# FlyCole/Dream2Real

Hardware: AMD Instinct MI355X
Metric: candidate renders scored/sec (640x360) (higher is better)
Workload: dtype bf16 + fp16 NeRF MLP operands (fp32 accumulate; the library's default: the reference's tiny-cuda-nn operand type, same MFMA rate; --opt mlp_f16=0 = bf16 operands)

## Files before the change

dream2real_amd/csrc/api.hip:

```cpp
#include <math.h>
#include <string.h>

#include <algorithm>
#include <chrono>

#include "d2r_internal.h"
#include "pngio.h"

struct d2r_clip;
int d2r_launch_preprocess(d2r_ctx *, d2r_clip *, const uint8_t *frames_dev, uint32_t n, uint32_t w, uint32_t h,
                          int rot90, uint16_t *patches_dev, float *pixel_values_dev, const void *rects_dev = nullptr,
                          const uint16_t *bg_patches_dev = nullptr, bool touched_only = false);
bool d2r_clip_l0_supported(const d2r_ctx *, const d2r_clip *);
int d2r_clip_forward(d2r_ctx *, const d2r_clip *, const uint16_t *patches_dev, uint32_t n, const float *text_dev,
                     uint32_t C, float logit_scale, float *logits_dev, float *embeds_dev, const ClipL0Reuse *reuse = nullptr);
int d2r_clip_layer0_background(d2r_ctx *, const d2r_clip *, const uint16_t *bg_patches_dev, ClipL0Reuse *out);
int d2r_launch_patchify(d2r_ctx *, const d2r_clip *, const float *pv_dev, uint32_t n, uint16_t *patches_dev);
size_t d2r_clip_patch_bytes(const d2r_clip *, uint32_t n);
int d2r_launch_eval_points(d2r_ctx *, const d2r_nerf *, const float *xyz, const float *dirs, uint32_t n, float *out);
uint32_t d2r_clip_image_size(const d2r_clip *);
uint32_t d2r_clip_proj_dim(const d2r_clip *);
uint32_t d2r_clip_max_images(const d2r_clip *);
uint32_t d2r_clip_tokens(const d2r_clip *);

// ... 104 lines not shown
    unsigned flags;
    int (*hook)(d2r_ctx *, int64_t value);
};
enum { OPT_DEV = 1,
       OPT_READ_ONLY = 2 };
#ifdef D2R_DEV
static const bool kDevBuild = true;
#else
static const bool kDevBuild = false;
#endif

static int opt_march_threads(d2r_ctx *ctx, int64_t value)
{
    if (value % 64)
        return d2r_fail(ctx, D2R_ERR_INVALID, "march_threads must be 0 (auto) or a multiple of 64 up to " + std::to_string(D2R_MARCH_THREADS) + " (the size the marcher was compiled for)");
    return D2R_OK;
}

static int opt_timing(d2r_ctx *ctx, int64_t)
{
    ctx->ev_used = 0;
    ctx->ev_pairs.clear();
    return D2R_OK;
}

static const Option g_options[] = {
    {"chunk", &d2r_ctx::chunk, Option::RANGE, 1, 16384},
    {"march_compact", &d2r_ctx::march_compact, Option::RANGE, 0, 1},
    {"refill_min", &d2r_ctx::refill_min, Option::RANGE, 1, 64},
    {"ln_fold", &d2r_ctx::ln_fold, Option::RANGE, 0, 4},
    {"gemm_nsplit", &d2r_ctx::gemm_nsplit, Option::FREE},
    {"prep_reuse", &d2r_ctx::prep_reuse, Option::FLAG},
    {"cls_last", &d2r_ctx::cls_last, Option::FLAG},
    {"vit_fp8", &d2r_ctx::vit_fp8, Option::FLAG},
    {"l0_reuse", &d2r_ctx::l0_reuse, Option::FLAG},
    {"attn_rem", &d2r_ctx::attn_rem, Option::RANGE, 0, 4},
    {"overlap", &d2r_ctx::overlap, Option::FLAG},
    {"debug_fail_chunk", &d2r_ctx::debug_fail_chunk, Option::FREE},
    {"ray_sort", &d2r_ctx::ray_sort, Option::RANGE, 0, 1},
    {"ray_sort_log2", &d2r_ctx::ray_sort_log2, Option::RANGE, 1, 4},
    {"march_threads", &d2r_ctx::march_threads, Option::RANGE, 0, D2R_MARCH_THREADS, 0, opt_march_threads},
    {"march_threads_auto_mib", &d2r_ctx::march_threads_auto_mib, Option::RANGE, 0, 1 << 20},
    {"march_blocks", &d2r_ctx::march_blocks, Option::RANGE, 0, 65535},
    {"gemm_cfg", &d2r_ctx::gemm_cfg, Option::FREE, 0, 0, OPT_DEV},
    {"gemm_group", &d2r_ctx::gemm_group, Option::RANGE, 0, 65535, OPT_DEV},
    {"gemm_stagger", &d2r_ctx::gemm_stagger, Option::FLAG, 0, 0, OPT_DEV},
    {"gbrick_slots", &d2r_ctx::gbrick_slots, Option::RANGE, 0, 8},
    {"brick_slots_total", &d2r_ctx::brick_slots_total, Option::RANGE, 0, 8},
    {"lds_slots_max", &d2r_ctx::lds_slots_max, Option::RANGE, 0, 5},
    {"gbrick_max_mib", &d2r_ctx::gbrick_max_mib, Option::RANGE, 0, 512},
    {"mlp_f16", &d2r_ctx::mlp_f16, Option::FLAG},
    {"render_arith", &d2r_ctx::render_arith, Option::RANGE, 0, 2},
    {"bricks", &d2r_ctx::use_bricks, Option::FLAG},
    {"raygen_rect", &d2r_ctx::raygen_rect, Option::FLAG},
    {"timing", &d2r_ctx::timing, Option::RANGE, 0, 2, 0, opt_timing},
    {"march_lds_slots", &d2r_ctx::last_march_nb, Option::FREE, 0, 0, OPT_READ_ONLY},
    {"march_hbm_brick_slots", &d2r_ctx::last_march_ngb, Option::FREE, 0, 0, OPT_READ_ONLY},
    {"march_hbm_brick_bytes", &d2r_ctx::last_march_gbrick_bytes, Option::FREE, 0, 0, OPT_READ_ONLY},
    {"march_threads_used", &d2r_ctx::last_march_threads, Option::FREE, 0, 0, OPT_READ_ONLY},
};

static const Option *find_option(const char *key)
{
    for (const Option &o : g_options)
        if (!strcmp(key, o.key)) return (o.flags & OPT_DEV) && !kDevBuild ? nullptr : &o;
    return nullptr;
// ... 948 lines not shown
```

dream2real_amd/csrc/clip.hip:

```cpp
#include "d2r_internal.h"

#include <type_traits>

#include <math.h>
#include <stdio.h>
#include <stdlib.h>

#include <algorithm>
#include <deque>
#include <mutex>

typedef __bf16 bf16x8 __attribute__((ext_vector_type(8)));
typedef float f32x16 __attribute__((ext_vector_type(16)));
typedef float f32x4 __attribute__((ext_vector_type(4)));

struct ClipWeights {
    const uint16_t *w_patch;
    const float *cls, *pos;
    const float *pre_w, *pre_b;
    struct Layer {
        const float *ln1_w, *ln1_b, *ln2_w, *ln2_b;
        const uint16_t *w_qkv, *w_o, *w_fc1, *w_fc2;
        const float *b_qkv, *b_o, *b_fc1, *b_fc2;
        const uint16_t *wf_qkv = nullptr, *wf_fc1 = nullptr;
// ... 2246 lines not shown
}

__global__ void k_gather_cls(const float *__restrict__ X, const uint16_t *__restrict__ Xhi, const uint16_t *__restrict__ Xlo,
                             uint32_t M_pad, uint32_t T, uint32_t d, uint32_t n, float *__restrict__ X_cls, int lo8 = 0)
{
    const uint32_t i = blockIdx.x * blockDim.x + threadIdx.x;
    if (i >= n * d) return;
    const uint32_t img = i / d, c = i - img * d;
    const size_t row = (size_t)img * T;
    float v;
    if (Xhi) {
        const size_t xo = ((size_t)(c >> 6) * M_pad + row) * 64 + (c & 63);
        v = __uint_as_float((uint32_t)Xhi[xo] << 16);
        if (Xlo && lo8) v = split8_value(Xhi[xo], ((const int8_t *)Xlo)[lo8_off(M_pad, row, c)]);
        else if (Xlo) v += __uint_as_float((uint32_t)Xlo[xo] << 16);
    } else {
        v = X[row * d + c];
    }
    X_cls[i] = v;
}

__global__ void k_gather_cls_operand(const uint16_t *__restrict__ Xhi, const float2 *__restrict__ AB, uint32_t M_pad, uint32_t T,
                                     uint32_t d, uint32_t n, uint16_t *__restrict__ Xq, float2 *__restrict__ ABq)
{
    const uint32_t i = blockIdx.x * blockDim.x + threadIdx.x, per = d / 8;
    if (i >= n * per) return;
    const uint32_t img = i / per, c = (i - img * per) * 8;
    const size_t row = (size_t)img * T;
    *(uint4 *)(Xq + (size_t)img * d + c) = *(const uint4 *)(Xhi + ((size_t)(c >> 6) * M_pad + row) * 64 + (c & 63));
    if (c == 0) ABq[img] = AB[row];
}


#define HEAD_THREADS 1024
#define HEAD_NI 4
__global__ __launch_bounds__(HEAD_THREADS) void k_head(const float *__restrict__ X, const uint16_t *__restrict__ Xb,
                                                       const uint16_t *__restrict__ Xlo, uint32_t M_pad,
                                                       const uint32_t *__restrict__ pool_row, uint32_t T, uint32_t d,
                                                       const float *__restrict__ lw, const float *__restrict__ lb,
                                                       const float *__restrict__ proj, uint32_t D,
                                                       const float *__restrict__ text, uint32_t C, float logit_scale,
                                                       float *__restrict__ logits, float *__restrict__ embeds, uint32_t n_items, int lo8 = 0)
{
    __shared__ float xs[HEAD_NI][1024];
    __shared__ float es[HEAD_NI][1024];
    __shared__ float red[HEAD_NI][16];
    constexpr uint32_t NW = HEAD_THREADS / 64;
    const uint32_t tid = threadIdx.x, lane = tid & 63, wave = tid >> 6;
    const uint32_t item0 = blockIdx.x * HEAD_NI;
    const uint32_t ni = min((uint32_t)HEAD_NI, n_items - item0);
    float xv[HEAD_NI];
#pragma unroll
    for (uint32_t m = 0; m < HEAD_NI; m++) {
        xv[m] = 0.f;
        if (m < ni && tid < d) {
            const size_t xrow = (size_t)(item0 + m) * T + (pool_row ? pool_row[item0 + m] : 0u);
            const size_t xo = ((size_t)(tid >> 6) * M_pad + xrow) * 64 + (tid & 63);
            xv[m] = Xb ? __uint_as_float((uint32_t)Xb[xo] << 16) : X[xrow * d + tid];
            if (Xb && Xlo && lo8) xv[m] = split8_value(Xb[xo], ((const int8_t *)Xlo)[lo8_off(M_pad, xrow, tid)]);
            else if (Xb && Xlo) xv[m] += __uint_as_float((uint32_t)Xlo[xo] << 16);
        }
        const float s = wave_sum(xv[m]);
        if (lane == 0) red[m][wave] = s;
    }
    __syncthreads();
    float mu[HEAD_NI], dv[HEAD_NI];
// ... 340 lines not shown
        if (g * 8 < n_qt) {
            if (r == 1) hipLaunchKernelGGL((k_attention_s<1, true>), dim3(n_heads, n, 1), dim3(64), lds, ctx->stream, QKV, AO, T, d, M_pad, g * 8, q8_scales);
            else if (r == 2) hipLaunchKernelGGL((k_attention_s<2, true>), dim3(n_heads, n, 1), dim3(128), lds, ctx->stream, QKV, AO, T, d, M_pad, g * 8, q8_scales);
            else hipLaunchKernelGGL((k_attention_s<4, true>), dim3(n_heads, n, 1), dim3(256), lds, ctx->stream, QKV, AO, T, d, M_pad, g * 8, q8_scales);
        }
        return;
    }
    if (g) hipLaunchKernelGGL((k_attention_s<8>), dim3(n_heads, n, g), dim3(512), lds, ctx->stream, QKV, AO, T, d, M_pad, 0u, no_scales);
    if (g * 8 < n_qt) {
        if (r == 1) hipLaunchKernelGGL((k_attention_s<1>), dim3(n_heads, n, 1), dim3(64), lds, ctx->stream, QKV, AO, T, d, M_pad, g * 8, no_scales);
        else if (r == 2) hipLaunchKernelGGL((k_attention_s<2>), dim3(n_heads, n, 1), dim3(128), lds, ctx->stream, QKV, AO, T, d, M_pad, g * 8, no_scales);
        else hipLaunchKernelGGL((k_attention_s<4>), dim3(n_heads, n, 1), dim3(256), lds, ctx->stream, QKV, AO, T, d, M_pad, g * 8, no_scales);
    }
}

static int attention_setup(d2r_ctx *ctx, uint32_t T_pad, size_t *lds_out)
{
    const size_t attn_lds = (size_t)T_pad * 128 + (size_t)64 * (T_pad + 4) * 2;
    if (attn_lds > 160 * 1024) return d2r_fail(ctx, D2R_ERR_UNSUPPORTED, "sequence too long for the resident attention LDS layout");
    static PerDeviceOnce attn_attr;
    attn_attr.run(ctx->device, [] {
        (void)hipFuncSetAttribute((const void *)k_attention<true>, hipFuncAttributeMaxDynamicSharedMemorySize, 160 * 1024);
    });
    *lds_out = attn_lds;
    return D2R_OK;
}

static int last_block_cls(d2r_ctx *ctx, const d2r_clip_desc &D, const ClipWeights::Layer &L, uint32_t n, uint32_t T, uint32_t rows_pad,
                          const uint16_t *QKV, const uint16_t *Qc, const float *X, const uint16_t *Xhi, const uint16_t *Xlo, float *Xc,
                          uint16_t *AOc, uint16_t *Xnc, uint16_t *Hc, int lo8 = 0)
{
    const uint32_t d = D.hidden_size, mlp = D.mlp_size, items = n * D.num_heads;
    int rc;
    hipLaunchKernelGGL(k_attention_cls, dim3((items + 3) / 4), dim3(256), 0, ctx->stream, QKV, Qc, AOc, T, d, rows_pad, D.num_heads, items);
    hipLaunchKernelGGL(k_gather_cls, dim3((n * d + 255) / 256), dim3(256), 0, ctx->stream, X, Xhi, Xlo, rows_pad, T, d, n, Xc, lo8);
    if ((rc = launch_gemm<EPI_BIAS_RESID_F32>(ctx, AOc, L.w_o, L.b_o, Xc, n, d, d))) return rc;
    hipLaunchKernelGGL(k_layernorm, dim3((n + 3) / 4), dim3(256), 0, ctx->stream, Xc, L.ln2_w, L.ln2_b, Xnc, n, d);
    if ((rc = launch_gemm<EPI_BIAS_GELU_BF16>(ctx, Xnc, L.w_fc1, L.b_fc1, Hc, n, mlp, d))) return rc;
    if ((rc = launch_gemm<EPI_BIAS_RESID_F32>(ctx, Hc, L.w_fc2, L.b_fc2, Xc, n, d, mlp))) return rc;
    return D2R_OK;
}

bool d2r_clip_l0_supported(const d2r_ctx *ctx, const d2r_clip *clip)
{
    const d2r_clip_desc &D = clip->desc;
    const uint32_t g = D.image_size / D.patch_size;
    return ctx->ln_fold == 4 && D.num_layers >= 2 && g * g == clip->T - 1 && g * g <= 1024;
}

int d2r_clip_layer0_background(d2r_ctx *ctx, const d2r_clip *clip, const uint16_t *bg_patches_dev, ClipL0Reuse *out)
{
    const d2r_clip_desc &D = clip->desc;
    const uint32_t d = D.hidden_size, T = clip->T, R = round_up(T, BM);
    if (T > 1025 || D.num_layers < 1) return d2r_fail(ctx, D2R_ERR_UNSUPPORTED, "layer-0 reuse needs at most 1024 patches per image");
    const size_t b_hi = (size_t)R * d * 2, b_lo = (size_t)R * d, b_ab = (size_t)R * 8, b_qkv = (size_t)R * 3 * d * 2, b_po = (size_t)R * d * 4;
    int rc;
    if ((rc = d2r_reserve(ctx, ctx->bg_l0, b_hi + b_lo + b_ab + b_qkv + b_po + 1024))) return rc;
    uint8_t *base = (uint8_t *)ctx->bg_l0.p;
    uint16_t *hi = (uint16_t *)base;
    uint8_t *lo = base + b_hi;
    float2 *ab = (float2 *)(lo + b_lo);
    uint16_t *qkv = (uint16_t *)((uint8_t *)ab + b_ab);
    float *po = (float *)((uint8_t *)qkv + b_qkv);
    if ((rc = launch_gemm<EPI_F32>(ctx, bg_patches_dev, clip->w.w_patch, nullptr, po, T - 1, d, clip->Kp_pad))) return rc;
    hipLaunchKernelGGL(k_embed_ln, dim3((T + 3) / 4), dim3(256), 0, ctx->stream, po, clip->w.cls, clip->w.pos, clip->w.pre_w, clip->w.pre_b,
                       (float *)nullptr, T, T, d, hi, ab, (uint16_t *)lo, R, 1);
    const ClipWeights::Layer &L = clip->layers[0];
// ... 44 lines not shown
        }
        f8[l].w_qkv = out[0]; f8[l].w_o = out[1]; f8[l].w_fc1 = out[2]; f8[l].w_fc2 = out[3];
    }
    std::vector<uint32_t> bits(nl * 4);
    D2R_HIP(ctx, hipMemcpyAsync(bits.data(), amax, nl * 16, hipMemcpyDeviceToHost, ctx->stream));
    D2R_HIP(ctx, hipStreamSynchronize(ctx->stream));
    auto scale_of = [](uint32_t b) {
        const int e = (int)((b + 0x200000u) >> 23);
        const int byte = std::min(std::max(e - 8, 1), 253);
        return std::ldexp(1.0f, byte - 127);
    };
    for (size_t l = 0; l < nl; l++) {
        f8[l].s_qkv = scale_of(bits[l * 4 + 0]); f8[l].s_o = scale_of(bits[l * 4 + 1]);
        f8[l].s_fc1 = scale_of(bits[l * 4 + 2]); f8[l].s_fc2 = scale_of(bits[l * 4 + 3]);
    }
    clip->f8 = std::move(f8);
    return D2R_OK;
}

int d2r_clip_forward(d2r_ctx *ctx, const d2r_clip *clip, const uint16_t *patches_dev, uint32_t n,
                     const float *text_dev, uint32_t C, float logit_scale, float *logits_dev, float *embeds_dev,
                     const ClipL0Reuse *reuse)
{
    const d2r_clip_desc &D = clip->desc;
    const uint32_t d = D.hidden_size, T = clip->T, mlp = D.mlp_size;
    const uint32_t rows = n * T, rows_pad = round_up(rows, BM);
    const uint32_t prow = n * (T - 1);
    int rc;
    if ((rc = d2r_reserve(ctx, ctx->clipws[0], (size_t)round_up(prow, BM) * d * 4))) return rc;
    if ((rc = d2r_reserve(ctx, ctx->clipws[1], (size_t)rows_pad * d * 4))) return rc;
    if ((rc = d2r_reserve(ctx, ctx->clipws[2], (size_t)rows_pad * d * 2))) return rc;
    if ((rc = d2r_reserve(ctx, ctx->clipws[3], (size_t)rows_pad * 3 * d * 2))) return rc;
    if ((rc = d2r_reserve(ctx, ctx->clipws[4], (size_t)rows_pad * d * 2))) return rc;
    if ((rc = d2r_reserve(ctx, ctx->clipws[5], (size_t)rows_pad * mlp * 2))) return rc;
    float *patch_out = (float *)ctx->clipws[0].p, *X = (float *)ctx->clipws[1].p;
    uint16_t *Xn = (uint16_t *)ctx->clipws[2].p, *QKV = (uint16_t *)ctx->clipws[3].p;
    uint16_t *AO = (uint16_t *)ctx->clipws[4].p, *H = (uint16_t *)ctx->clipws[5].p;

    const int fold = (int)ctx->ln_fold;
    const bool l0 = reuse && reuse->rects;
    if (l0 && (!d2r_clip_l0_supported(ctx, clip) || T > reuse->bg_rows))
        return d2r_fail(ctx, D2R_ERR_INVALID, "d2r_clip_forward: layer-0 reuse requested for a model / option set that does not support it");
    uint32_t *l0_cnt = nullptr, *l0_list = nullptr;
    const uint32_t cap_pad = round_up(prow, BM);
    if (l0) {
        const PrepCache *pc = nullptr;
        if ((rc = prep_tables(ctx, (d2r_clip *)clip, reuse->w, reuse->h, 1, &pc))) return rc;
        if ((rc = d2r_reserve(ctx, ctx->l0_misc, 256 + (size_t)prow * 4 + (size_t)cap_pad * 8))) return rc;
        if ((rc = d2r_reserve(ctx, ctx->l0_a1, (size_t)cap_pad * clip->Kp_pad * 2))) return rc;
        if ((rc = d2r_reserve(ctx, ctx->l0_q2, (size_t)cap_pad * 3 * d * 2))) return rc;
        l0_cnt = (uint32_t *)ctx->l0_misc.p;
        l0_list = l0_cnt + 64;
        D2R_HIP(ctx, hipMemsetAsync(l0_cnt, 0, 4, ctx->stream));
        hipLaunchKernelGGL(k_touch_list, dim3(n), dim3(256), 0, ctx->stream, (const int4 *)reuse->rects, reuse->w, pc->R, D.image_size, D.patch_size, l0_cnt, l0_list);
        hipLaunchKernelGGL(k_gather_rows, dim3(2048), dim3(256), 0, ctx->stream, patches_dev, clip->Kp_pad, l0_list, l0_cnt, (uint16_t *)ctx->l0_a1.p);
        if (reuse->touched_out) D2R_HIP(ctx, hipMemcpyAsync(reuse->touched_out, l0_cnt, 4, hipMemcpyDeviceToDevice, ctx->stream));
        if (getenv("D2R_L0_DEBUG")) {
            uint32_t c = 0;
            (void)hipMemcpyAsync(&c, l0_cnt, 4, hipMemcpyDeviceToHost, ctx->stream);
            (void)hipStreamSynchronize(ctx->stream);
            fprintf(stderr, "[d2r l0_reuse] %u of %u patch tokens touched (%.1f %%)\n", c, prow, 100.0 * c / prow);
        }
        EpiAux a1{};
        a1.m_dev = l0_cnt;
        if ((rc = launch_gemm_cfg<EPI_F32, 4, 2, 2, 3>(ctx, (const uint16_t *)ctx->l0_a1.p, clip->w.w_patch, nullptr, patch_out, prow, d, clip->Kp_pad, a1))) return rc;
    } else if ((rc = launch_gemm<EPI_F32>(ctx, patches_dev, clip->w.w_patch, nullptr, patch_out, prow, d, clip->Kp_pad)))
        return rc;
// ... 3 lines not shown
    a_tm.a_rs = 64;
    a_tm.a_ks = (uint32_t)64 * rows_pad;
    if ((uint64_t)64 * rows_pad >= (1ull << 32)) return d2r_fail(ctx, D2R_ERR_UNSUPPORTED, "activation plane too large for 32-bit indexing");
    if (fold == 0) {
        hipLaunchKernelGGL(k_embed_ln, dim3((rows + 3) / 4), dim3(256), 0, ctx->stream, patch_out, clip->w.cls,
                           clip->w.pos, clip->w.pre_w, clip->w.pre_b, X, rows, T, d, (uint16_t *)nullptr, (float2 *)nullptr, (uint16_t *)nullptr, rows_pad);
        for (uint32_t l = 0; l < D.num_layers; l++) {
            const ClipWeights::Layer &L = clip->layers[l];
            hipLaunchKernelGGL(k_layernorm, dim3((rows + 3) / 4), dim3(256), 0, ctx->stream, X, L.ln1_w, L.ln1_b, Xn,
                               rows, d);
            if ((rc = launch_gemm<EPI_BIAS_BF16>(ctx, Xn, L.w_qkv, L.b_qkv, QKV, rows, 3 * d, d, out_tm))) return rc;
            if (cls_last && l + 1 == D.num_layers) {
                if ((rc = last_block_cls(ctx, D, L, n, T, rows_pad, QKV, nullptr, X, nullptr, nullptr, patch_out, AO, Xn, H))) return rc;
                break;
            }
            launch_attention_vision(ctx, QKV, AO, T, d, rows_pad, D.num_heads, n);
            if ((rc = launch_gemm<EPI_BIAS_RESID_F32>(ctx, AO, L.w_o, L.b_o, X, rows, d, d, a_tm))) return rc;
            hipLaunchKernelGGL(k_layernorm, dim3((rows + 3) / 4), dim3(256), 0, ctx->stream, X, L.ln2_w, L.ln2_b, Xn,
                               rows, d);
            if ((rc = launch_gemm<EPI_BIAS_GELU_BF16>(ctx, Xn, L.w_fc1, L.b_fc1, H, rows, mlp, d, out_tm))) return rc;
            if ((rc = launch_gemm<EPI_BIAS_RESID_F32>(ctx, H, L.w_fc2, L.b_fc2, X, rows, d, mlp, a_tm))) return rc;
        }
        hipLaunchKernelGGL(k_head, dim3((n + HEAD_NI - 1) / HEAD_NI), dim3(HEAD_THREADS), 0, ctx->stream, cls_last ? patch_out : X, (const uint16_t *)nullptr, (const uint16_t *)nullptr, rows_pad,
                           (const uint32_t *)nullptr, cls_last ? 1u : T, d,
                           clip->w.post_w, clip->w.post_b, clip->w.proj, D.proj_dim, text_dev, C, logit_scale, logits_dev, embeds_dev, n);
        D2R_HIP(ctx, hipGetLastError());
        return D2R_OK;
    }
    const uint32_t np = d / 64;
    if ((rc = d2r_reserve(ctx, ctx->clipws[7], (size_t)rows_pad * np * 8 + (size_t)rows_pad * 8))) return rc;
    float2 *part = (float2 *)ctx->clipws[7].p, *AB = part + (size_t)rows_pad * np;
    const bool xf32 = fold == 3, split8 = fold == 4, split = fold == 1 || split8;
    const int lo8 = split8 ? 1 : 0;
    uint16_t *Xlo = split ? (uint16_t *)X : (uint16_t *)nullptr;
    if (l0) {
        hipLaunchKernelGGL(k_bcast_x0, dim3((rows + 3) / 4), dim3(256), 0, ctx->stream, reuse->bg_hi, reuse->bg_lo, reuse->bg_ab, reuse->bg_rows, Xn,
                           (uint8_t *)Xlo, AB, rows, rows_pad, T, d);
        hipLaunchKernelGGL(k_embed_ln, dim3(std::min<uint32_t>((prow + 3) / 4, 4096u)), dim3(256), 0, ctx->stream, patch_out, clip->w.cls, clip->w.pos, clip->w.pre_w,
                           clip->w.pre_b, (float *)nullptr, rows, T, d, Xn, AB, Xlo, rows_pad, lo8, (const uint32_t *)l0_list, (const uint32_t *)l0_cnt);
    } else
    hipLaunchKernelGGL(k_embed_ln, dim3((rows + 3) / 4), dim3(256), 0, ctx->stream, patch_out, clip->w.cls, clip->w.pos,
                       clip->w.pre_w, clip->w.pre_b, xf32 ? X : (float *)nullptr, rows, T, d, Xn, AB, Xlo, rows_pad, lo8);
    EpiAux ln = out_tm, st = a_tm;
    ln.a_rs = a_tm.a_rs;
    ln.a_ks = a_tm.a_ks;
    ln.ab = AB;
    st.hm_rows = rows_pad;
    st.xb = Xn;
    st.part = part;
    st.xlo = Xlo;
    const float inv_d = 1.0f / (float)d;
    uint32_t f8_first = D.num_layers, f8_end = D.num_layers;
    uint8_t *A8 = nullptr, *SA8 = nullptr, *AOS8 = nullptr, *H8 = nullptr, *SH8 = nullptr;
    uint32_t q8_grid = 0;
    if (ctx->vit_fp8 && split8 && d % 256 == 0 && mlp % 256 == 0 && mlp >= 2 * d) {
        f8_first = l0 ? 1u : 0u;
        f8_end = cls_last ? D.num_layers - 1 : D.num_layers;
        if (f8_first < f8_end) {
            if ((rc = ensure_f8_weights(ctx, (d2r_clip *)clip))) return rc;
            const size_t rp = rows_pad;
            AOS8 = (uint8_t *)AO + rp * d;
            H8 = (uint8_t *)H;
            SH8 = H8 + rp * mlp;
            A8 = SH8 + rp * (mlp / 64);
            SA8 = A8 + rp * d;
            q8_grid = (uint32_t)ctx->n_cu * 8u;
        }
    }
    for (uint32_t l = 0; l < D.num_layers; l++) {
        const ClipWeights::Layer &L = clip->layers[l];
        ln.cs = L.cs_qkv;
        if (cls_last && l + 1 == D.num_layers) {
            EpiAux kv = ln;
            kv.cs = L.cs_qkv + d;
            if ((rc = launch_gemm<EPI_LN_BIAS_BF16>(ctx, Xn, L.wf_qkv + (size_t)d * d, L.bf_qkv + d, QKV + (size_t)d * rows_pad, rows, 2 * d, d, kv)))
                return rc;
            const uint32_t n_pad = round_up(n, BM);
            uint16_t *Xq = H, *Qc = H + (size_t)n_pad * d;
            float2 *ABq = part;
            hipLaunchKernelGGL(k_gather_cls_operand, dim3((n * (d / 8) + 255) / 256), dim3(256), 0, ctx->stream, Xn, AB, rows_pad, T, d, n, Xq, ABq);
            EpiAux lq{};
            lq.cs = L.cs_qkv;
            lq.ab = ABq;
            if ((rc = launch_gemm<EPI_LN_BIAS_BF16>(ctx, Xq, L.wf_qkv, L.bf_qkv, Qc, n, d, d, lq))) return rc;
            if ((rc = last_block_cls(ctx, D, L, n, T, rows_pad, QKV, Qc, X, xf32 ? nullptr : Xn, Xlo, patch_out, AO, Xn, H, lo8))) return rc;
            break;
        }
        if (f8_first <= l && l < f8_end) {
            const d2r_clip::F8Layer &F = clip->f8[l];
            hipLaunchKernelGGL(k_ln_q8, dim3(q8_grid), dim3(256), 0, ctx->stream, Xn, AB, L.ln1_w, L.ln1_b, rows_pad, d, A8, SA8);
            if ((rc = launch_gemm_f8<EPI_F8_BIAS_BF16>(ctx, A8, SA8, F.w_qkv, F.s_qkv, L.b_qkv, QKV, rows, 3 * d, d, out_tm))) return rc;
            launch_attention_vision(ctx, QKV, AO, T, d, rows_pad, D.num_heads, n, AOS8);
            if ((rc = launch_gemm_f8<EPI_F8_RESID_STATS_SPLIT8>(ctx, (const uint8_t *)AO, AOS8, F.w_o, F.s_o, L.b_o, Xn, rows, d, d, st))) return rc;
            hipLaunchKernelGGL(k_rowstats, dim3((rows_pad + 255) / 256), dim3(256), 0, ctx->stream, part, np, rows_pad, inv_d, AB);
            hipLaunchKernelGGL(k_ln_q8, dim3(q8_grid), dim3(256), 0, ctx->stream, Xn, AB, L.ln2_w, L.ln2_b, rows_pad, d, A8, SA8);
            EpiAux hq = out_tm;
            hq.q8 = H8;
            hq.q8_scale = SH8;
            if ((rc = launch_gemm_f8<EPI_F8_BIAS_GELU_Q8>(ctx, A8, SA8, F.w_fc1, F.s_fc1, L.b_fc1, nullptr, rows, mlp, d, hq))) return rc;
            if ((rc = launch_gemm_f8<EPI_F8_RESID_STATS_SPLIT8>(ctx, H8, SH8, F.w_fc2, F.s_fc2, L.b_fc2, Xn, rows, d, mlp, st))) return rc;
            if (l + 1 < D.num_layers)
                hipLaunchKernelGGL(k_rowstats, dim3((rows_pad + 255) / 256), dim3(256), 0, ctx->stream, part, np, rows_pad, inv_d, AB);
            continue;
        }
        if (l0 && l == 0) {
            const uint32_t planes = 3 * d / 64;
            const size_t pieces = (size_t)planes * rows * 8;
            hipLaunchKernelGGL(k_bcast_qkv, dim3((uint32_t)((pieces + 255) / 256)), dim3(256), 0, ctx->stream, reuse->bg_qkv, reuse->bg_rows, QKV, rows, rows_pad, T, planes);
            float2 *AB2 = (float2 *)((uint8_t *)ctx->l0_misc.p + 256 + (size_t)prow * 4);
            hipLaunchKernelGGL(k_gather_operand_rows, dim3(2048), dim3(256), 0, ctx->stream, Xn, AB, rows_pad, T, (const uint32_t *)l0_list, (const uint32_t *)l0_cnt,
                               AO, AB2, cap_pad, d);
            EpiAux l2 = ln;
            l2.a_ks = 64 * cap_pad;
            l2.hm_rows = cap_pad;
            l2.ab = AB2;
            l2.m_dev = l0_cnt;
            if ((rc = launch_gemm_cfg<EPI_LN_BIAS_BF16, 4, 2, 2, 3>(ctx, AO, L.wf_qkv, L.bf_qkv, ctx->l0_q2.p, prow, 3 * d, d, l2))) return rc;
            hipLaunchKernelGGL(k_scatter_qkv, dim3(8192), dim3(256), 0, ctx->stream, (const uint16_t *)ctx->l0_q2.p, cap_pad, (const uint32_t *)l0_list,
// ... 407 lines not shown
```

dream2real_amd/csrc/d2r_internal.h:

```cpp
#pragma once
#include <hip/hip_runtime.h>
#include <stdint.h>

#include <functional>
#include <memory>
#include <mutex>
#include <string>
#include <utility>
#include <vector>

#include "../../include/d2r.h"
#include "d2r_shared.h"

class D2rJobPool;
struct D2rPngBase;

#define D2R_MAX_LEVELS 16
#define D2R_MAX_DEVICES 64
#define D2R_GRID 128
#define D2R_DT 0.0016914558f
#define D2R_INV_DT (1.0f / D2R_DT)
#define D2R_CONE 0.00390625f
#define D2R_T_LINEAR (D2R_DT * 256.0f)
#define D2R_N_WFRAG 24
// ... 102 lines not shown
    uint32_t bg_w = 0, bg_h = 0;
    d2r_render_stats stats{};
    int n_cu = 256, n_xcd = 8;
    void *comm = nullptr;
    int comm_rank = 0, comm_world = 1;
    hipStream_t render_stream = nullptr, copy_stream = nullptr;
    hipEvent_t ev_fork = nullptr, ev_prep[2] = {nullptr, nullptr}, ev_clip[2] = {nullptr, nullptr},
               ev_march[2] = {nullptr, nullptr}, ev_copy[2] = {nullptr, nullptr};
    Buf patches2, frames2;
    void *frame_host[2] = {nullptr, nullptr};
    size_t frame_host_cap[2] = {0, 0};
    D2rJobPool *pool = nullptr;
    std::shared_ptr<const D2rPngBase> png_base;
    int64_t overlap = 0;
    int64_t debug_fail_chunk = -1;
    uint32_t last_chunks = 0;
    int64_t chunk = 4096;
    uint32_t last_pass = 0;
    int64_t march_blocks = 0;
    int64_t ray_sort = 1;
    int64_t ray_sort_log2 = 4;
    int64_t march_threads = 0;
    int64_t march_threads_auto_mib = 64;
    int64_t last_march_threads = 0, last_march_gbrick_bytes = 0;
    int64_t last_march_nb = 0, last_march_ngb = 0;
    int64_t refill_min = 64;
    int64_t march_compact = 1;
    int64_t ln_fold = 4;
    int64_t gemm_stagger = 0;
    int64_t gemm_group = 65535;
    int64_t gemm_nsplit = 0;
    int64_t attn_rem = 1;
    int64_t cls_last = 1;
    int64_t gemm_cfg = 0;
    int64_t mlp_f16 = 1;
    int64_t render_arith = 0;
    int64_t use_bricks = 1;
    int64_t raygen_rect = 1;
    int64_t gbrick_slots = 8;
    int64_t brick_slots_total = 7;
    int64_t lds_slots_max = 5;
    int64_t gbrick_max_mib = 512;
    int64_t timing = 0;
    std::vector<hipEvent_t> ev_pool;
    size_t ev_used = 0;
    std::vector<std::pair<int, std::pair<size_t, size_t>>> ev_pairs;
    size_t timing_begin(int kind);
    void timing_end(size_t pair);
};
enum { D2R_T_MARCH = 0, D2R_T_RAYGEN = 1, D2R_T_CLIP = 2, D2R_T_PREP = 3, D2R_T_SORT = 4,
       D2R_T_VIT_QKV = 5, D2R_T_VIT_ATTN = 6, D2R_T_VIT_OUT = 7, D2R_T_VIT_FC1 = 8, D2R_T_VIT_FC2 = 9, D2R_T_KINDS = 10 };

struct d2r_nerf {
    d2r_ctx *ctx;
    int device = 0;
    NerfParams P{};
    D2rDev<uint32_t> d_grid, d_brick_tab, d_gbrick_tab;
    D2rDev<uint64_t> d_bricks;
    D2rDev<uint4> d_wfrag;
};

struct d2r_pcd {
    int device = 0;
    uint32_t n = 0;
    D2rDev<float4> xyz;
    D2rDev<uint32_t> rgb;
// ... 42 lines not shown
```

Measured before the change: 28870.

## Fold K/V projections into CLS-only last-layer attention to skip full KV GEMM

In the last ViT layer, when only the CLS token is needed, the full K/V projection over all tokens is skipped. The CLS query is folded through the K weights into a per-head query in hidden space. Attention scores and the probability-weighted token sum are then computed directly on the normalized hidden states, and the V projection is applied once per head afterwards. This removes a large rows×2d×d GEMM in exchange for three new kernels that carry fp32 values as hi/lo bf16 splits to preserve precision, plus a larger workspace.

```diff
diff --git a/dream2real_amd/csrc/api.hip b/dream2real_amd/csrc/api.hip
--- a/dream2real_amd/csrc/api.hip
+++ b/dream2real_amd/csrc/api.hip
@@ -160,6 +160,7 @@
     {"gemm_nsplit", &d2r_ctx::gemm_nsplit, Option::FREE},
     {"prep_reuse", &d2r_ctx::prep_reuse, Option::FLAG},
     {"cls_last", &d2r_ctx::cls_last, Option::FLAG},
+    {"cls_fold", &d2r_ctx::cls_fold, Option::FLAG},
     {"vit_fp8", &d2r_ctx::vit_fp8, Option::FLAG},
     {"l0_reuse", &d2r_ctx::l0_reuse, Option::FLAG},
     {"attn_rem", &d2r_ctx::attn_rem, Option::RANGE, 0, 4},
diff --git a/dream2real_amd/csrc/clip.hip b/dream2real_amd/csrc/clip.hip
--- a/dream2real_amd/csrc/clip.hip
+++ b/dream2real_amd/csrc/clip.hip
@@ -2302,6 +2302,312 @@
 }
 
 
+#define CLSF_NI 8
+__global__ __launch_bounds__(256) void k_cls_qfold(const uint16_t *__restrict__ Qc, const uint16_t *__restrict__ Wk, const float *__restrict__ csk,
+                                                   uint32_t n, uint32_t d, uint32_t H, float *__restrict__ Qt, float *__restrict__ Cc)
+{
+    __shared__ __attribute__((aligned(16))) float qs[64][CLSF_NI];
+    const uint32_t h = blockIdx.y, i0 = blockIdx.x * CLSF_NI, tid = threadIdx.x, lane = tid & 63, np2 = d >> 1;
+    for (uint32_t idx = tid; idx < 64 * CLSF_NI; idx += 256) {
+        const uint32_t i = idx >> 6, e = idx & 63;
+        qs[e][i] = i0 + i < n ? __uint_as_float((uint32_t)Qc[(size_t)(i0 + i) * d + h * 64 + e] << 16) : 0.f;
+    }
+    __syncthreads();
+    if (tid < 64) {
+        const float cs = csk[h * 64 + lane];
+#pragma unroll
+        for (int i = 0; i < CLSF_NI; i++) {
+            const float v = wave_sum(qs[lane][i] * cs);
+            if (lane == 0 && i0 + i < n) Cc[(size_t)(i0 + i) * H + h] = v;
+        }
+    }
+    float acc[2][CLSF_NI][2];
+#pragma unroll
+    for (int t = 0; t < 2; t++)
+#pragma unroll
+        for (int i = 0; i < CLSF_NI; i++) acc[t][i][0] = acc[t][i][1] = 0.f;
+    const uint16_t *Wh = Wk + (size_t)h * 64 * d;
+#pragma unroll 4
+    for (uint32_t e = 0; e < 64; e++) {
+        const float4 qa = *(const float4 *)&qs[e][0], qb = *(const float4 *)&qs[e][4];
+        const float q[CLSF_NI] = {qa.x, qa.y, qa.z, qa.w, qb.x, qb.y, qb.z, qb.w};
+#pragma unroll
+        for (int t = 0; t < 2; t++) {
+            const uint32_t pi = tid + 256 * t;
+            if (pi < np2) {
+                const uint32_t wv = *(const uint32_t *)(Wh + (size_t)e * d + 2 * pi);
+                const float w0 = bf_lo(wv), w1 = bf_hi(wv);
+#pragma unroll
+                for (int i = 0; i < CLSF_NI; i++) {
+                    acc[t][i][0] = fmaf(q[i], w0, acc[t][i][0]);
+                    acc[t][i][1] = fmaf(q[i], w1, acc[t][i][1]);
+                }
+            }
+        }
+    }
+#pragma unroll
+    for (int t = 0; t < 2; t++) {
+        const uint32_t pi = tid + 256 * t;
+        if (pi >= np2) continue;
+#pragma unroll
+        for (int i = 0; i < CLSF_NI; i++)
+            if (i0 + i < n) *(float2 *)(Qt + ((size_t)(i0 + i) * H + h) * d + 2 * pi) = make_float2(acc[t][i][0], acc[t][i][1]);
+    }
+}
+
+static size_t cls_fold_lds(uint32_t d, uint32_t nw) { return (size_t)32 * (d + 8) * 2 + (size_t)nw * 2 * 64 * 16 + 32 * 16 * 4 + 2 * 16 * 4 + 4 * 16 * 4 + 16 * 4; }
+
+__global__ __launch_bounds__(512) void k_attention_cls_fold(const uint16_t *__restrict__ Xn, const float2 *__restrict__ AB,
+                                                            const float *__restrict__ Qt, const float *__restrict__ Cc, uint32_t T, uint32_t d,
+                                                            uint32_t M_pad, uint32_t H, float *__restrict__ P, float *__restrict__ SB)
+{
+    extern __shared__ __attribute__((aligned(16))) uint8_t cf_lds[];
+    const uint32_t tid = threadIdx.x, lane = tid & 63, w = tid >> 6, NT = blockDim.x, NW = NT >> 6, img = blockIdx.x;
+    const uint32_t xst = d + 8;
+    uint16_t *xs = (uint16_t *)cf_lds;
+    float4 *part = (float4 *)(xs + 32 * xst);
+    float *wl = (float *)(part + NW * 128);
+    float *tmax = wl + 512;
+    float *red = tmax + 32;
+    float *scb = red + 64;
+    const uint32_t hb = 4 * (lane >> 4), tl = lane & 15, kq = 8 * (lane >> 4);
+    const uint32_t KS = d >> 5, NP = 4 * d;
+    const size_t row0 = (size_t)img * T;
+    union U8 { uint4 u; bf16x8 v; };
+    bf16x8 qhi[4], qlo[4];
+#pragma unroll
+    for (int i = 0; i < 4; i++) {
+        const uint32_t kk = 4 * w + i;
+        float4 v0 = make_float4(0.f, 0.f, 0.f, 0.f), v1 = v0;
+        if (kk < KS && tl < H) {
+            const float *qp = Qt + ((size_t)img * H + tl) * d + kk * 32 + kq;
+            v0 = *(const float4 *)qp;
+            v1 = *(const float4 *)(qp + 4);
+        }
+        const uint32_t h0 = pack2(v0.x, v0.y), h1 = pack2(v0.z, v0.w), h2 = pack2(v1.x, v1.y), h3 = pack2(v1.z, v1.w);
+        U8 th, tq;
+        th.u = make_uint4(h0, h1, h2, h3);
+        tq.u = make_uint4(pack2(v0.x - bf_lo(h0), v0.y - bf_hi(h0)), pack2(v0.z - bf_lo(h1), v0.w - bf_hi(h1)),
+                          pack2(v1.x - bf_lo(h2), v1.y - bf_hi(h2)), pack2(v1.z - bf_lo(h3), v1.w - bf_hi(h3)));
+        qhi[i] = th.v;
+        qlo[i] = tq.v;
+    }
+    float ch[4];
+#pragma unroll
+    for (int r = 0; r < 4; r++) ch[r] = hb + r < H ? Cc[(size_t)img * H + hb + r] : 0.f;
+    float acc0[16], acc1[16];
+#pragma unroll
+    for (int h = 0; h < 16; h++) { acc0[h] = 0.f; acc1[h] = 0.f; }
+    float mine[4], ls[4], lb[4];
+#pragma unroll
+    for (int r = 0; r < 4; r++) { mine[r] = -INFINITY; ls[r] = 0.f; lb[r] = 0.f; }
+    const bool colok = tid < (d >> 1);
+    typedef unsigned u32x4 __attribute__((ext_vector_type(4)));
+    u32x4 pf[8];
+    f32x2 abn[2] = {f32x2{0.f, 0.f}, f32x2{0.f, 0.f}};
+#define CLS_FOLD_ISSUE(C0)                                                                                                             \
+    {                                                                                                                                  \
+        _Pragma("unroll") for (int i = 0; i < 8; i++) {                                                                                \
+            const uint32_t idx = tid + i * NT;                                                                                         \
+            if (idx < NP)                                                                                                              \
+                pf[i] = *(const u32x4 *)(Xn +((size_t)(idx >> 8) * M_pad + row0 + min((C0) + ((idx >> 3) & 31), T - 1)) * 64 + (idx & 7) * 8); \
+        }                                                                                                                              \
+        if (w < 2) abn[0] = *(const f32x2 *)(AB + row0 + min((C0) + 16 * w + tl, T - 1));                                              \
+        if (w + NW < 2) abn[1] = *(const f32x2 *)(AB + row0 + min((C0) + 16 * (w + NW) + tl, T - 1));                                  \
+    }
+    CLS_FOLD_ISSUE(0u)
+    for (uint32_t c0 = 0; c0 < T; c0 += 32) {
+#pragma unroll
+        for (int i = 0; i < 8; i++) {
+            const uint32_t idx = tid + i * NT;
+            if (idx < NP) *(u32x4 *)(xs + ((idx >> 3) & 31) * xst + (idx >> 8) * 64 + (idx & 7) * 8) = pf[i];
+        }
+        const float2 ab[2] = {make_float2(abn[0][0], abn[0][1]), make_float2(abn[1][0], abn[1][1])};
+        __syncthreads();
+        if (c0 + 32 < T) CLS_FOLD_ISSUE(c0 + 32)
+#pragma unroll
+        for (int tile = 0; tile < 2; tile++) {
+            f32x4 sh = {0.f, 0.f, 0.f, 0.f}, sl = sh;
+            if (c0 + 16 * tile < T) {
+                const uint16_t *bp = xs + (16 * tile + tl) * xst + kq;
+#pragma unroll
+                for (int i = 0; i < 4; i++) {
+                    const uint32_t kk = 4 * w + i;
+                    if (kk < KS) {
+                        U8 x;
+                        x.u = *(const uint4 *)(bp + kk * 32);
+                        sh = __builtin_amdgcn_mfma_f32_16x16x32_bf16(qhi[i], x.v, sh, 0, 0, 0);
+                        sl = __builtin_amdgcn_mfma_f32_16x16x32_bf16(qlo[i], x.v, sl, 0, 0, 0);
+                    }
+                }
+            }
+            part[(w * 2 + tile) * 64 + lane] = make_float4(sh[0] + sl[0], sh[1] + sl[1], sh[2] + sl[2], sh[3] + sl[3]);
+        }
+        __syncthreads();
+        float s[2][4];
+#pragma unroll
+        for (int ti = 0; ti < 2; ti++) {
+            const uint32_t tile = w + ti * NW;
+#pragma unroll
+            for (int r = 0; r < 4; r++) s[ti][r] = -INFINITY;
+            if (tile < 2) {
+                float4 S = part[tile * 64 + lane];
+                for (uint32_t ww = 1; ww < NW; ww++) {
+                    const float4 o = part[(ww * 2 + tile) * 64 + lane];
+                    S = make_float4(S.x + o.x, S.y + o.y, S.z + o.z, S.w + o.w);
+                }
+                const float Sv[4] = {S.x, S.y, S.z, S.w};
+                float tm[4];
+#pragma unroll
+                for (int r = 0; r < 4; r++) {
+                    if (c0 + 16 * tile + tl < T) s[ti][r] = fmaf(ab[ti].x, Sv[r], ab[ti].y * ch[r]);
+                    tm[r] = s[ti][r];
+#pragma unroll
+                    for (int o = 1; o < 16; o <<= 1) tm[r] = fmaxf(tm[r], __shfl_xor(tm[r], o));
+                }
+                if (tl == 0) *(float4 *)(tmax + tile * 16 + hb) = make_float4(tm[0], tm[1], tm[2], tm[3]);
+            }
+        }
+        __syncthreads();
+        if (w < 2) {
+            const float4 t0 = *(const float4 *)(tmax + hb), t1 = *(const float4 *)(tmax + 16 + hb);
+            const float mxs[4] = {fmaxf(t0.x, t1.x), fmaxf(t0.y, t1.y), fmaxf(t0.z, t1.z), fmaxf(t0.w, t1.w)};
+            float mn[4], scl[4];
+#pragma unroll
+            for (int r = 0; r < 4; r++) {
+                mn[r] = fmaxf(mine[r], mxs[r]);
+                scl[r] = __builtin_amdgcn_exp2f(mine[r] - mn[r]);
+                mine[r] = mn[r];
+                ls[r] *= scl[r];
+                lb[r] *= scl[r];
+            }
+            if (w == 0 && tl == 0) *(float4 *)(scb + hb) = make_float4(scl[0], scl[1], scl[2], scl[3]);
+#pragma unroll
+            for (int ti = 0; ti < 2; ti++) {
+                const uint32_t tile = w + ti * NW;
+                if (tile >= 2) continue;
+                float wv[4];
+#pragma unroll
+                for (int r = 0; r < 4; r++) {
+                    const float p = __builtin_amdgcn_exp2f(s[ti][r] - mn[r]);
+                    ls[r] += p;
+                    lb[r] = fmaf(p, ab[ti].y, lb[r]);
+                    wv[r] = p * ab[ti].x;
+                }
+                *(float4 *)(wl + (16 * tile + tl) * 16 + hb) = make_float4(wv[0], wv[1], wv[2], wv[3]);
+            }
+        }
+        __syncthreads();
+        if (colok) {
+            const uint32_t nj = min(32u, T - c0);
+#pragma unroll
+            for (int g = 0; g < 4; g++) {
+                const float4 sc = *(const float4 *)(scb + 4 * g);
+                acc0[4 * g + 0] *= sc.x; acc1[4 * g + 0] *= sc.x; acc0[4 * g + 1] *= sc.y; acc1[4 * g + 1] *= sc.y;
+                acc0[4 * g + 2] *= sc.z; acc1[4 * g + 2] *= sc.z; acc0[4 * g + 3] *= sc.w; acc1[4 * g + 3] *= sc.w;
+            }
+            const uint16_t *xp = xs + 2 * tid;
+#pragma unroll 1
+            for (uint32_t jj = 0; jj < nj; jj++) {
+                const uint32_t xv = *(const uint32_t *)(xp + jj * xst);
+                const float x0 = bf_lo(xv), x1 = bf_hi(xv);
+#pragma unroll
+                for (int g = 0; g < 4; g++) {
+                    if (4u * g >= H) continue;
+                    const float4 wv = *(const float4 *)(wl + jj * 16 + 4 * g);
+                    acc0[4 * g + 0] = fmaf(wv.x, x0, acc0[4 * g + 0]); acc1[4 * g + 0] = fmaf(wv.x, x1, acc1[4 * g + 0]);
+                    acc0[4 * g + 1] = fmaf(wv.y, x0, acc0[4 * g + 1]); acc1[4 * g + 1] = fmaf(wv.y, x1, acc1[4 * g + 1]);
+                    acc0[4 * g + 2] = fmaf(wv.z, x0, acc0[4 * g + 2]); acc1[4 * g + 2] = fmaf(wv.z, x1, acc1[4 * g + 2]);
+                    acc0[4 * g + 3] = fmaf(wv.w, x0, acc0[4 * g + 3]); acc1[4 * g + 3] = fmaf(wv.w, x1, acc1[4 * g + 3]);
+                }
+            }
+        }
+        __syncthreads();
+    }
+    const uint32_t NF = min(NW, 2u);
+    if (w < 2) {
+#pragma unroll
+        for (int r = 0; r < 4; r++)
+#pragma unroll
+            for (int o = 1; o < 16; o <<= 1) {
+                ls[r] += __shfl_xor(ls[r], o);
+                lb[r] += __shfl_xor(lb[r], o);
+            }
+        if (tl == 0) {
+            *(float4 *)(red + (w * 2 + 0) * 16 + hb) = make_float4(ls[0], ls[1], ls[2], ls[3]);
+            *(float4 *)(red + (w * 2 + 1) * 16 + hb) = make_float4(lb[0], lb[1], lb[2], lb[3]);
+        }
+    }
+    __syncthreads();
+    if (colok) {
+#pragma unroll
+        for (int g = 0; g < 4; g++) {
+            if (4u * g >= H) continue;
+            float4 l = *(const float4 *)(red + 4 * g);
+            if (NF > 1) {
+                const float4 o = *(const float4 *)(red + 32 + 4 * g);
+                l = make_float4(l.x + o.x, l.y + o.y, l.z + o.z, l.w + o.w);
+            }
+            const float inv[4] = {1.0f / l.x, 1.0f / l.y, 1.0f / l.z, 1.0f / l.w};
+#pragma unroll
+            for (int r = 0; r < 4; r++)
+                if (4u * g + r < H)
+                    *(float2 *)(P + ((size_t)img * H + 4 * g + r) * d + 2 * tid) = make_float2(acc0[4 * g + r] * inv[r], acc1[4 * g + r] * inv[r]);
+        }
+    }
+    if (tid < H) {
+        float l = red[tid], b = red[16 + tid];
+        if (NF > 1) {
+            l += red[32 + tid];
+            b += red[48 + tid];
+        }
+        SB[(size_t)img * H + tid] = b / l;
+    }
+#undef CLS_FOLD_ISSUE
+}
+
+__global__ __launch_bounds__(256) void k_cls_ofold(const float *__restrict__ P, const float *__restrict__ SB, const uint16_t *__restrict__ Wv,
+                                                   const float *__restrict__ csv, const float *__restrict__ bfv, uint32_t n, uint32_t d, uint32_t H,
+                                                   uint16_t *__restrict__ AOc)
+{
+    const uint32_t h = blockIdx.y, lane = threadIdx.x & 63, w = threadIdx.x >> 6, tl = lane & 15, kq = 8 * (lane >> 4), hb = 4 * (lane >> 4);
+    const uint32_t i0 = (blockIdx.x * 4 + w) * 16;
+    if (i0 >= n) return;
+    const float *pp = P + ((size_t)min(i0 + tl, n - 1) * H + h) * d + kq;
+    const uint16_t *wp = Wv + (size_t)(h * 64 + tl) * d + kq;
+    union U8 { uint4 u; bf16x8 v; };
+    f32x4 acc[4];
+#pragma unroll
+    for (int et = 0; et < 4; et++) acc[et] = f32x4{0.f, 0.f, 0.f, 0.f};
+    for (uint32_t kk = 0; kk < (d >> 5); kk++) {
+        const float4 v0 = *(const float4 *)(pp + kk * 32), v1 = *(const float4 *)(pp + kk * 32 + 4);
+        const uint32_t h0 = pack2(v0.x, v0.y), h1 = pack2(v0.z, v0.w), h2 = pack2(v1.x, v1.y), h3 = pack2(v1.z, v1.w);
+        U8 ahi, alo;
+        ahi.u = make_uint4(h0, h1, h2, h3);
+        alo.u = make_uint4(pack2(v0.x - bf_lo(h0), v0.y - bf_hi(h0)), pack2(v0.z - bf_lo(h1), v0.w - bf_hi(h1)),
+                           pack2(v1.x - bf_lo(h2), v1.y - bf_hi(h2)), pack2(v1.z - bf_lo(h3), v1.w - bf_hi(h3)));
+#pragma unroll
+        for (int et = 0; et < 4; et++) {
+            U8 x;
+            x.u = *(const uint4 *)(wp + (size_t)et * 16 * d + kk * 32);
+            acc[et] = __builtin_amdgcn_mfma_f32_16x16x32_bf16(ahi.v, x.v, acc[et], 0, 0, 0);
+            acc[et] = __builtin_amdgcn_mfma_f32_16x16x32_bf16(alo.v, x.v, acc[et], 0, 0, 0);
+        }
+    }
+    float sb[4];
+#pragma unroll
+    for (int r = 0; r < 4; r++) sb[r] = i0 + hb + r < n ? SB[(size_t)(i0 + hb + r) * H + h] : 0.f;
+#pragma unroll
+    for (int et = 0; et < 4; et++) {
+        const uint32_t col = h * 64 + et * 16 + tl;
+        const float cs = csv[col], bf = bfv[col];
+#pragma unroll
+        for (int r = 0; r < 4; r++)
+            if (i0 + hb + r < n) AOc[(size_t)(i0 + hb + r) * d + col] = f2bf(fmaf(sb[r], cs, acc[et][r]) + bf);
+    }
+}
+
+
 #define HEAD_THREADS 1024
 #define HEAD_NI 4
 __global__ __launch_bounds__(HEAD_THREADS) void k_head(const float *__restrict__ X, const uint16_t *__restrict__ Xb,
@@ -2708,7 +3014,8 @@
 {
     const uint32_t d = D.hidden_size, mlp = D.mlp_size, items = n * D.num_heads;
     int rc;
-    hipLaunchKernelGGL(k_attention_cls, dim3((items + 3) / 4), dim3(256), 0, ctx->stream, QKV, Qc, AOc, T, d, rows_pad, D.num_heads, items);
+    if (QKV)
+        hipLaunchKernelGGL(k_attention_cls, dim3((items + 3) / 4), dim3(256), 0, ctx->stream, QKV, Qc, AOc, T, d, rows_pad, D.num_heads, items);
     hipLaunchKernelGGL(k_gather_cls, dim3((n * d + 255) / 256), dim3(256), 0, ctx->stream, X, Xhi, Xlo, rows_pad, T, d, n, Xc, lo8);
     if ((rc = launch_gemm<EPI_BIAS_RESID_F32>(ctx, AOc, L.w_o, L.b_o, Xc, n, d, d))) return rc;
     hipLaunchKernelGGL(k_layernorm, dim3((n + 3) / 4), dim3(256), 0, ctx->stream, Xc, L.ln2_w, L.ln2_b, Xnc, n, d);
@@ -2819,7 +3126,8 @@
     if ((rc = d2r_reserve(ctx, ctx->clipws[2], (size_t)rows_pad * d * 2))) return rc;
     if ((rc = d2r_reserve(ctx, ctx->clipws[3], (size_t)rows_pad * 3 * d * 2))) return rc;
     if ((rc = d2r_reserve(ctx, ctx->clipws[4], (size_t)rows_pad * d * 2))) return rc;
-    if ((rc = d2r_reserve(ctx, ctx->clipws[5], (size_t)rows_pad * mlp * 2))) return rc;
+    const size_t fold_ws = (size_t)round_up(n, BM) * d * 4 + ((size_t)2 * n * D.num_heads * d + 2 * (size_t)round_up(n * D.num_heads, 4u)) * 4;
+    if ((rc = d2r_reserve(ctx, ctx->clipws[5], std::max((size_t)rows_pad * mlp * 2, fold_ws)))) return rc;
     float *patch_out = (float *)ctx->clipws[0].p, *X = (float *)ctx->clipws[1].p;
     uint16_t *Xn = (uint16_t *)ctx->clipws[2].p, *QKV = (uint16_t *)ctx->clipws[3].p;
     uint16_t *AO = (uint16_t *)ctx->clipws[4].p, *H = (uint16_t *)ctx->clipws[5].p;
@@ -2889,6 +3197,7 @@
     float2 *part = (float2 *)ctx->clipws[7].p, *AB = part + (size_t)rows_pad * np;
     const bool xf32 = fold == 3, split8 = fold == 4, split = fold == 1 || split8;
     const int lo8 = split8 ? 1 : 0;
+    const bool cls_fold = cls_last && ctx->cls_fold && !xf32 && d <= 1024 && d == 64 * D.num_heads;
     uint16_t *Xlo = split ? (uint16_t *)X : (uint16_t *)nullptr;
     if (l0) {
         hipLaunchKernelGGL(k_bcast_x0, dim3((rows + 3) / 4), dim3(256), 0, ctx->stream, reuse->bg_hi, reuse->bg_lo, reuse->bg_ab, reuse->bg_rows, Xn,
@@ -2928,10 +3237,12 @@
         const ClipWeights::Layer &L = clip->layers[l];
         ln.cs = L.cs_qkv;
         if (cls_last && l + 1 == D.num_layers) {
-            EpiAux kv = ln;
-            kv.cs = L.cs_qkv + d;
-            if ((rc = launch_gemm<EPI_LN_BIAS_BF16>(ctx, Xn, L.wf_qkv + (size_t)d * d, L.bf_qkv + d, QKV + (size_t)d * rows_pad, rows, 2 * d, d, kv)))
-                return rc;
+            if (!cls_fold) {
+                EpiAux kv = ln;
+                kv.cs = L.cs_qkv + d;
+                if ((rc = launch_gemm<EPI_LN_BIAS_BF16>(ctx, Xn, L.wf_qkv + (size_t)d * d, L.bf_qkv + d, QKV + (size_t)d * rows_pad, rows, 2 * d, d, kv)))
+                    return rc;
+            }
             const uint32_t n_pad = round_up(n, BM);
             uint16_t *Xq = H, *Qc = H + (size_t)n_pad * d;
             float2 *ABq = part;
@@ -2940,7 +3251,21 @@
             lq.cs = L.cs_qkv;
             lq.ab = ABq;
             if ((rc = launch_gemm<EPI_LN_BIAS_BF16>(ctx, Xq, L.wf_qkv, L.bf_qkv, Qc, n, d, d, lq))) return rc;
-            if ((rc = last_block_cls(ctx, D, L, n, T, rows_pad, QKV, Qc, X, xf32 ? nullptr : Xn, Xlo, patch_out, AO, Xn, H, lo8))) return rc;
+            if (cls_fold) {
+                const uint32_t Hh = D.num_heads, nw = round_up(d / 2, 64u) / 64;
+                float *Qt = (float *)(H + (size_t)2 * n_pad * d), *Pl = Qt + (size_t)n * Hh * d;
+                float *Cc = Pl + (size_t)n * Hh * d, *Sb = Cc + (size_t)round_up(n * Hh, 4u);
+                const size_t lds = cls_fold_lds(d, nw);
+                static PerDeviceOnce fold_attr;
+                fold_attr.run(ctx->device, [] {
+                    (void)hipFuncSetAttribute((const void *)k_attention_cls_fold, hipFuncAttributeMaxDynamicSharedMemorySize, (int)cls_fold_lds(1024, 8));
+                });
+                hipLaunchKernelGGL(k_cls_qfold, dim3((n + CLSF_NI - 1) / CLSF_NI, Hh), dim3(256), 0, ctx->stream, Qc, L.wf_qkv + (size_t)d * d, L.cs_qkv + d, n, d, Hh, Qt, Cc);
+                hipLaunchKernelGGL(k_attention_cls_fold, dim3(n), dim3(nw * 64), lds, ctx->stream, Xn, AB, Qt, Cc, T, d, rows_pad, Hh, Pl, Sb);
+                hipLaunchKernelGGL(k_cls_ofold, dim3((n + 63) / 64, Hh), dim3(256), 0, ctx->stream, Pl, Sb, L.wf_qkv + (size_t)2 * d * d, L.cs_qkv + 2 * d,
+                                   L.bf_qkv + 2 * d, n, d, Hh, AO);
+            }
+            if ((rc = last_block_cls(ctx, D, L, n, T, rows_pad, cls_fold ? nullptr : QKV, Qc, X, xf32 ? nullptr : Xn, Xlo, patch_out, AO, Xn, H, lo8))) return rc;
             break;
         }
         if (f8_first <= l && l < f8_end) {
diff --git a/dream2real_amd/csrc/d2r_internal.h b/dream2real_amd/csrc/d2r_internal.h
--- a/dream2real_amd/csrc/d2r_internal.h
+++ b/dream2real_amd/csrc/d2r_internal.h
@@ -158,6 +158,7 @@
     int64_t gemm_nsplit = 0;
     int64_t attn_rem = 1;
     int64_t cls_last = 1;
+    int64_t cls_fold = 1;
     int64_t gemm_cfg = 0;
     int64_t mlp_f16 = 1;
     int64_t render_arith = 0;
```

Result: no change. 28940, median of 6 (+0.3%).
